# cheneeheng/2s-AGCN

Measured on AMD Instinct MI355X. Metric: skeleton-clips/sec fwd+bwd, NTU (N,3,300,25,2), higher is better.
Workload: dtype f32; 1 GPU; AGCN joint-stream NTU-xview shape, full training step (fwd, CE, bwd, grad all-reduce, clip 1.0, SGD nesterov); per_gpu_batch=64, global_batch=64, input=(N,3,300,25,2), parallelism=dp1, bn=per-replica

## Files before the change

2s-agcn_amd/csrc/wgrad9_bf16.hip:

```cpp
#include "agcn_common.h"
#include "split_bf16.h"
#include "split_f16.h"

namespace {

constexpr int TC = 80;
constexpr int DP = 84;
constexpr int XW = TC + 8;
constexpr int XPB = 88;

struct TrArgs {
  const float* in;
  float* out;
  int N, R, T, V, Tp, S;
  const float* absmax;
  long plane;
};

template <bool F16, int RB, int TT, int FPL>
__global__ void __launch_bounds__(256) tv_transpose_kernel(const TrArgs a) {
  extern __shared__ __attribute__((aligned(16))) float tile[];
  static_assert(FPL == 4 || (F16 && FPL == 8), "a lane writes one 16-byte store per plane");
  constexpr int QL = TT / FPL, NSUB = 64 / QL;
  const int S = a.S;
  const int ntt = (a.Tp * S + TT - 1) / TT, nrb = (a.R + RB - 1) / RB;
  int b = blockIdx.x;
  const int tti = b % ntt;
  b /= ntt;
  const int rb = b % nrb, n = b / nrb;
  const int t0 = tti * TT, r0 = rb * RB;
  const int tl = max(0, min(TT, a.T - t0));
  const int len = tl * a.V;
  const int pitch = TT * a.V + 4;
  const int lane = threadIdx.x & 63;
  const int wave = __builtin_amdgcn_readfirstlane(threadIdx.x >> 6);
  typedef const __attribute__((address_space(1))) void* gptr_t;
  typedef __attribute__((address_space(3))) void* lptr_t;
  const bool wide = ((a.T * a.V) & 3) == 0 && (len & 3) == 0 && len > 0 && ((reinterpret_cast<unsigned long>(a.in) & 15) == 0);
  if (wide) {
    const int npiece = (len + 255) >> 8;
    for (int p = wave; p < RB * npiece; p += 4) {
      const int r = p / npiece, e0 = (p - r * npiece) * 256;
      if (r0 + r < a.R) {
        const float* src = a.in + (((long)n * a.R + r0 + r) * a.T + t0) * a.V + e0;
        if (e0 + 4 * lane < len)
          __builtin_amdgcn_global_load_lds((gptr_t)(src + 4 * lane), (lptr_t)(tile + r * pitch + e0), 16, 0, 0);
      }
    }
  } else {
    const int npiece = (len + 63) >> 6;
    for (int p = wave; p < RB * npiece; p += 4) {
      const int r = p / npiece, e0 = (p - r * npiece) * 64;
      if (r0 + r < a.R) {
        const float* src = a.in + (((long)n * a.R + r0 + r) * a.T + t0) * a.V + e0;
        const int e = min(lane, len - 1 - e0);
        __builtin_amdgcn_global_load_lds((gptr_t)(src + e), (lptr_t)(tile + r * pitch + e0), 4, 0, 0);
      }
    }
  }
  __syncthreads();
  float rs_s = 1.f, rs_inv = 1.f;
  if constexpr (F16) f16_range_scale(a.absmax, rs_s, rs_inv);
  (void)rs_inv;
  const int TTo = TT / S;
  const int tw = min(TTo, a.Tp - t0 / S);
  const int qp = TTo / FPL;
  const int lq = lane % QL;
  const int par = lq / qp, q = lq - par * qp, sub = lane / QL;
  for (int p = wave * NSUB + sub; p < a.V * RB; p += 4 * NSUB) {
    const int v = p / RB, r = p - v * RB;
    if (r0 + r < a.R && FPL * q < tw) {
      float val[FPL];
#pragma unroll
      for (int j = 0; j < FPL; ++j) {
        const int f = (FPL * q + j) * S + par;
        val[j] = (f < tl) ? tile[r * pitch + f * a.V + v] : 0.f;
      }
      const long o = ((((long)n * a.V + v) * a.R + r0 + r) * S + par) * a.Tp + t0 / S + FPL * q;
      if constexpr (F16) {
        unsigned hh[FPL / 2], ll[FPL / 2];
#pragma unroll
        for (int j = 0; j < FPL / 2; ++j) split_pair_f16_mix(val[2 * j] * rs_s, val[2 * j + 1] * rs_s, hh[j], ll[j]);
        unsigned short* oh = reinterpret_cast<unsigned short*>(a.out);
        if constexpr (FPL == 8) {
          *reinterpret_cast<u32x4*>(oh + o) = u32x4{hh[0], hh[1], hh[2], hh[3]};
          *reinterpret_cast<u32x4*>(oh + a.plane + o) = u32x4{ll[0], ll[1], ll[2], ll[3]};
        } else {
          *reinterpret_cast<uint2*>(oh + o) = make_uint2(hh[0], hh[1]);
          *reinterpret_cast<uint2*>(oh + a.plane + o) = make_uint2(ll[0], ll[1]);
        }
      } else {
        *reinterpret_cast<f32x4*>(a.out + o) = f32x4{val[0], val[1], val[2], val[3]};
      }
    }
  }
}

struct W9Args {
  const float* dyT;
  const float* xT;
  float* part;
  int N, M, C, V, T, Tp;
  int nchunk, units, units_per_split, ncb;
  int npl;
  const unsigned short* dyH;
  const unsigned short* xH;
  long dy_plane, x_plane;
  const float* dy_absmax;
  const float* x_absmax;
};

template <int S>
__device__ __forceinline__ bf16x8 window_frag(const unsigned (&p)[8]) {
  u32x4 r;
  if (S % 2 == 0) {
#pragma unroll
    for (int i = 0; i < 4; ++i) r[i] = p[S / 2 + i];
  } else {
#pragma unroll
    for (int i = 0; i < 4; ++i) r[i] = __builtin_amdgcn_alignbit(p[(S + 1) / 2 + i], p[(S - 1) / 2 + i], 16);
  }
  return __builtin_bit_cast(bf16x8, r);
}

template <int S>
__device__ __forceinline__ f32x16 tap_mfma(bf16x8 a0, bf16x8 a1, bf16x8 a2, const unsigned (&p0)[8],
                                           const unsigned (&p1)[8], const unsigned (&p2)[8], f32x16 c, int npl) {
  return sb_mfma6(a0, a1, a2, window_frag<S>(p0), window_frag<S>(p1), window_frag<S>(p2), c, npl);
}

template <int RT, int CT, int STRIDE>
__global__ void __launch_bounds__(256, 2) wgrad9_bf16_kernel(const W9Args a) {
  constexpr int NT = 256, BM = RT * 32, CBW = CT * 32, SETS = STRIDE;
  static_assert(RT * CT == 4, "four waves");
  constexpr int ND = BM * (TC / 4) / NT;
  constexpr int NXG = CBW * SETS * (XW / 8);
  constexpr int NX = (NXG + NT - 1) / NT;
  static_assert(BM * (TC / 4) % NT == 0, "dy tile divides evenly");
  extern __shared__ __attribute__((aligned(16))) float smem[];
  float* dyL = smem;
  unsigned short* xP = reinterpret_cast<unsigned short*>(smem + BM * DP);
  const int tid = threadIdx.x, lane = tid & 63;
  const int wave = __builtin_amdgcn_readfirstlane(tid >> 6);
  const int lr = lane & 31, h = lane >> 5;
  const int rt = wave % RT, ct = wave / RT;
  const int mb = blockIdx.x / a.ncb, cb = blockIdx.x - mb * a.ncb;
  const int m0 = mb * BM, c0 = cb * CBW;
  const int split = blockIdx.y;
  const int u_begin = split * a.units_per_split;
  const int u_end = min(a.units, u_begin + a.units_per_split);
  const int Tp = a.Tp;

  f32x16 acc[9];
#pragma unroll
  for (int z = 0; z < 9; ++z)
#pragma unroll
    for (int j = 0; j < 16; ++j) acc[z][j] = 0.f;

  const float* arow = dyL + (rt * 32 + lr) * DP + 8 * h;
  const unsigned short* brow = xP + (ct * 32 + lr) * XPB + 8 * h;

  for (int unit = u_begin; unit < u_end; ++unit) {
    const int ch = unit % a.nchunk;
    const int nv = unit / a.nchunk;
    const int t0 = ch * TC;
    const float* src = a.dyT + ((long)nv * a.M + m0) * Tp + t0;
    const float* sx = a.xT + ((long)nv * a.C + c0) * SETS * Tp + (t0 - 4);
    int tv = tid;
    asm volatile("" : "+v"(tv));
    f32x4 dv[ND], xv[NX][2];
#pragma unroll
    for (int u = 0; u < ND; ++u) {
      const int i = tv + u * NT, r = i / (TC / 4), q = i - r * (TC / 4);
      const bool ok = (m0 + r < a.M) && (t0 + 4 * q < Tp);
      dv[u] = *reinterpret_cast<const f32x4*>(src + (ok ? r * Tp + 4 * q : 0));
      if (!ok) dv[u] = f32x4{0.f, 0.f, 0.f, 0.f};
    }
#pragma unroll
    for (int u = 0; u < NX; ++u) {
      const int i = min(tv + u * NT, NXG - 1), r = i / (XW / 8), k = i - r * (XW / 8);
#pragma unroll
      for (int hq = 0; hq < 2; ++hq) {
        const int t = t0 - 4 + 8 * k + 4 * hq;
        const bool ok = (c0 + r / SETS < a.C) && t >= 0 && t < Tp;
        xv[u][hq] = *reinterpret_cast<const f32x4*>(sx + (ok ? r * Tp + 8 * k + 4 * hq : 4));
        if (!ok) xv[u][hq] = f32x4{0.f, 0.f, 0.f, 0.f};
      }
    }
    __syncthreads();
    asm volatile("" : "+v"(tv));
#pragma unroll
    for (int u = 0; u < ND; ++u) {
      const int i = tv + u * NT, r = i / (TC / 4), q = i - r * (TC / 4);
      *reinterpret_cast<f32x4*>(dyL + r * DP + 4 * q) = dv[u];
    }
#pragma unroll
    for (int u = 0; u < NX; ++u) {
      const int i = min(tv + u * NT, NXG - 1), r = i / (XW / 8), k = i - r * (XW / 8);
      u32x4 ph, pm, pl;
#pragma unroll
      for (int e = 0; e < 4; ++e) {
        unsigned y0, y1, y2;
        sb_split_pair(xv[u][e >> 1][2 * (e & 1)], xv[u][e >> 1][2 * (e & 1) + 1], y0, y1, y2);
        ph[e] = y0; pm[e] = y1; pl[e] = y2;
      }
      const int row = (r % SETS) * CBW + r / SETS;
      *reinterpret_cast<u32x4*>(xP + (0 * SETS * CBW + row) * XPB + 8 * k) = ph;
      *reinterpret_cast<u32x4*>(xP + (1 * SETS * CBW + row) * XPB + 8 * k) = pm;
      *reinterpret_cast<u32x4*>(xP + (2 * SETS * CBW + row) * XPB + 8 * k) = pl;
    }
    __syncthreads();
#pragma unroll 1
    for (int ks = 0; ks < TC / 16; ++ks) {
      const f32x4 ar0 = *reinterpret_cast<const f32x4*>(arow + 16 * ks);
      const f32x4 ar1 = *reinterpret_cast<const f32x4*>(arow + 16 * ks + 4);
      u32x4 bw[SETS][3][2];
#pragma unroll
      for (int st = 0; st < SETS; ++st)
#pragma unroll
        for (int pl = 0; pl < 3; ++pl)
#pragma unroll
          for (int i = 0; i < 2; ++i)
            bw[st][pl][i] = *reinterpret_cast<const u32x4*>(brow + (pl * SETS + st) * CBW * XPB + 16 * ks + 8 * i);
      u32x4 ah, am, al;
      {
        unsigned x0, x1, x2;
        sb_split_pair(ar0[0], ar0[1], x0, x1, x2); ah[0] = x0; am[0] = x1; al[0] = x2;
        sb_split_pair(ar0[2], ar0[3], x0, x1, x2); ah[1] = x0; am[1] = x1; al[1] = x2;
        sb_split_pair(ar1[0], ar1[1], x0, x1, x2); ah[2] = x0; am[2] = x1; al[2] = x2;
        sb_split_pair(ar1[2], ar1[3], x0, x1, x2); ah[3] = x0; am[3] = x1; al[3] = x2;
      }
      unsigned p0[8], p1[8], p2[8], o0[8], o1[8], o2[8];
#pragma unroll
      for (int i = 0; i < 8; ++i) {
        p0[i] = bw[0][0][i >> 2][i & 3];
        p1[i] = bw[0][1][i >> 2][i & 3];
        p2[i] = bw[0][2][i >> 2][i & 3];
        o0[i] = bw[SETS - 1][0][i >> 2][i & 3];
        o1[i] = bw[SETS - 1][1][i >> 2][i & 3];
        o2[i] = bw[SETS - 1][2][i >> 2][i & 3];
      }
      const bf16x8 a0 = __builtin_bit_cast(bf16x8, ah), a1 = __builtin_bit_cast(bf16x8, am),
                   a2 = __builtin_bit_cast(bf16x8, al);
      if (STRIDE == 1) {
        acc[0] = tap_mfma<0>(a0, a1, a2, p0, p1, p2, acc[0], a.npl);
        acc[1] = tap_mfma<1>(a0, a1, a2, p0, p1, p2, acc[1], a.npl);
        acc[2] = tap_mfma<2>(a0, a1, a2, p0, p1, p2, acc[2], a.npl);
        acc[3] = tap_mfma<3>(a0, a1, a2, p0, p1, p2, acc[3], a.npl);
        acc[4] = tap_mfma<4>(a0, a1, a2, p0, p1, p2, acc[4], a.npl);
        acc[5] = tap_mfma<5>(a0, a1, a2, p0, p1, p2, acc[5], a.npl);
        acc[6] = tap_mfma<6>(a0, a1, a2, p0, p1, p2, acc[6], a.npl);
        acc[7] = tap_mfma<7>(a0, a1, a2, p0, p1, p2, acc[7], a.npl);
        acc[8] = tap_mfma<8>(a0, a1, a2, p0, p1, p2, acc[8], a.npl);
      } else {
        acc[0] = tap_mfma<2>(a0, a1, a2, p0, p1, p2, acc[0], a.npl);
        acc[1] = tap_mfma<2>(a0, a1, a2, o0, o1, o2, acc[1], a.npl);
        acc[2] = tap_mfma<3>(a0, a1, a2, p0, p1, p2, acc[2], a.npl);
        acc[3] = tap_mfma<3>(a0, a1, a2, o0, o1, o2, acc[3], a.npl);
        acc[4] = tap_mfma<4>(a0, a1, a2, p0, p1, p2, acc[4], a.npl);
        acc[5] = tap_mfma<4>(a0, a1, a2, o0, o1, o2, acc[5], a.npl);
        acc[6] = tap_mfma<5>(a0, a1, a2, p0, p1, p2, acc[6], a.npl);
        acc[7] = tap_mfma<5>(a0, a1, a2, o0, o1, o2, acc[7], a.npl);
        acc[8] = tap_mfma<6>(a0, a1, a2, p0, p1, p2, acc[8], a.npl);
      }
    }
  }

  float* dst = a.part + (long)split * 9 * a.M * a.C;
#pragma unroll
  for (int z = 0; z < 9; ++z)
#pragma unroll
    for (int j = 0; j < 16; ++j) {
      const int m = m0 + rt * 32 + mfma_row(j, h);
      const int c = c0 + ct * 32 + lr;
      if (m < a.M && c < a.C) dst[((long)z * a.M + m) * a.C + c] = acc[z][j];
    }
}


constexpr int DPH = 88;

template <int S>
__device__ __forceinline__ f32x16 tap_mfma_f16(f16x8 ah, f16x8 al, const unsigned (&ph)[8], const unsigned (&pl)[8],
                                               f32x16 c) {
  const f16x8 bh = __builtin_bit_cast(f16x8, window_frag<S>(ph)), bl = __builtin_bit_cast(f16x8, window_frag<S>(pl));
  c = __builtin_amdgcn_mfma_f32_32x32x16_f16(al, bh, c, 0, 0, 0);
  c = __builtin_amdgcn_mfma_f32_32x32x16_f16(ah, bl, c, 0, 0, 0);
  c = __builtin_amdgcn_mfma_f32_32x32x16_f16(ah, bh, c, 0, 0, 0);
  return c;
}

template <int RT, int CT, int STRIDE, int TAPS = 9, int SH0 = 0>
__global__ void __launch_bounds__(256, 2) wgrad9_f16_kernel(const W9Args a) {
  static_assert(STRIDE == 1 || (TAPS == 9 && SH0 == 0), "other tap counts at stride 1 only");
  static_assert(SH0 >= 0 && SH0 + TAPS - 1 <= 8, "every tap's 8 frames lie inside the 16-frame window");
  constexpr int NT = 256, BM = RT * 32, CBW = CT * 32, SETS = STRIDE;
  static_assert(RT * CT == 4, "four waves");
  constexpr int ND = BM * (TC / 4) / NT;
  constexpr int NXG = CBW * SETS * (XW / 8);
  constexpr int NX = (NXG + NT - 1) / NT;
  static_assert(BM * (TC / 4) % NT == 0, "dy tile divides evenly");
  extern __shared__ __attribute__((aligned(16))) unsigned short smh[];
  unsigned short* dyL = smh;
  unsigned short* xP = smh + 2 * BM * DPH;
  const int tid = threadIdx.x, lane = tid & 63;
  const int wave = __builtin_amdgcn_readfirstlane(tid >> 6);
  const int lr = lane & 31, h = lane >> 5;
  const int rt = wave % RT, ct = wave / RT;
  const int mb = blockIdx.x / a.ncb, cb = blockIdx.x - mb * a.ncb;
  const int m0 = mb * BM, c0 = cb * CBW;
  const int split = blockIdx.y;
  const int u_begin = split * a.units_per_split;
  const int u_end = min(a.units, u_begin + a.units_per_split);
  const int Tp = a.Tp;

  f32x16 acc[9];
#pragma unroll
  for (int z = 0; z < 9; ++z)
#pragma unroll
    for (int j = 0; j < 16; ++j) acc[z][j] = 0.f;

  const unsigned short* arow = dyL + (rt * 32 + lr) * DPH + 8 * h;
  const unsigned short* brow = xP + (ct * 32 + lr) * XPB + 8 * h;

  constexpr bool PREF = STRIDE == 1;
  uint2 dv[ND][2], xv[NX][2][2];
  auto fetch = [&](int unit) __attribute__((always_inline)) {
    const int ch = unit % a.nchunk;
    const int nv = unit / a.nchunk;
    const int t0 = ch * TC;
    const unsigned short* src = a.dyH + ((long)nv * a.M + m0) * Tp + t0;
    const unsigned short* sx = a.xH + ((long)nv * a.C + c0) * SETS * Tp + (t0 - 4);
    int tv = tid;
    asm volatile("" : "+v"(tv));
#pragma unroll
    for (int u = 0; u < ND; ++u) {
      const int i = tv + u * NT, r = i / (TC / 4), q = i - r * (TC / 4);
      const bool ok = (m0 + r < a.M) && (t0 + 4 * q < Tp);
      const int off = ok ? r * Tp + 4 * q : 0;
#pragma unroll
      for (int pl = 0; pl < 2; ++pl) {
        dv[u][pl] = *reinterpret_cast<const uint2*>(src + pl * a.dy_plane + off);
        if (!ok) dv[u][pl] = make_uint2(0u, 0u);
      }
    }
#pragma unroll
    for (int u = 0; u < NX; ++u) {
      const int i = min(tv + u * NT, NXG - 1), r = i / (XW / 8), k = i - r * (XW / 8);
#pragma unroll
      for (int hq = 0; hq < 2; ++hq) {
        const int t = t0 - 4 + 8 * k + 4 * hq;
        const bool ok = (c0 + r / SETS < a.C) && t >= 0 && t < Tp;
        const int off = ok ? r * Tp + 8 * k + 4 * hq : 4;
#pragma unroll
        for (int pl = 0; pl < 2; ++pl) {
          xv[u][hq][pl] = *reinterpret_cast<const uint2*>(sx + pl * a.x_plane + off);
          if (!ok) xv[u][hq][pl] = make_uint2(0u, 0u);
        }
      }
    }
  };
  if (PREF && u_begin < u_end) fetch(u_begin);
  for (int unit = u_begin; unit < u_end; ++unit) {
    if (!PREF) fetch(unit);
    __syncthreads();
    int tv = tid;
    asm volatile("" : "+v"(tv));
#pragma unroll
    for (int u = 0; u < ND; ++u) {
      const int i = tv + u * NT, r = i / (TC / 4), q = i - r * (TC / 4);
#pragma unroll
      for (int pl = 0; pl < 2; ++pl) *reinterpret_cast<uint2*>(dyL + (pl * BM + r) * DPH + 4 * q) = dv[u][pl];
    }
#pragma unroll
    for (int u = 0; u < NX; ++u) {
      const int i = min(tv + u * NT, NXG - 1), r = i / (XW / 8), k = i - r * (XW / 8);
      const int row = (r % SETS) * CBW + r / SETS;
#pragma unroll
      for (int hq = 0; hq < 2; ++hq)
#pragma unroll
        for (int pl = 0; pl < 2; ++pl)
          *reinterpret_cast<uint2*>(xP + (pl * SETS * CBW + row) * XPB + 8 * k + 4 * hq) = xv[u][hq][pl];
    }
    __syncthreads();
    if (PREF && unit + 1 < u_end) fetch(unit + 1);
#pragma unroll 1
    for (int ks = 0; ks < TC / 16; ++ks) {
      const f16x8 ah = *reinterpret_cast<const f16x8*>(arow + 16 * ks);
      const f16x8 al = *reinterpret_cast<const f16x8*>(arow + BM * DPH + 16 * ks);
      u32x4 bw[SETS][2][2];
#pragma unroll
      for (int st = 0; st < SETS; ++st)
#pragma unroll
        for (int pl = 0; pl < 2; ++pl)
#pragma unroll
          for (int i = 0; i < 2; ++i)
            bw[st][pl][i] = *reinterpret_cast<const u32x4*>(brow + (pl * SETS + st) * CBW * XPB + 16 * ks + 8 * i);
      unsigned p0[8], p1[8], o0[8], o1[8];
#pragma unroll
      for (int i = 0; i < 8; ++i) {
        p0[i] = bw[0][0][i >> 2][i & 3];
        p1[i] = bw[0][1][i >> 2][i & 3];
        o0[i] = bw[SETS - 1][0][i >> 2][i & 3];
        o1[i] = bw[SETS - 1][1][i >> 2][i & 3];
      }
      if constexpr (STRIDE == 1) {
        acc[0] = tap_mfma_f16<SH0 + 0>(ah, al, p0, p1, acc[0]);
        if constexpr (TAPS > 1) acc[1] = tap_mfma_f16<SH0 + 1>(ah, al, p0, p1, acc[1]);
        if constexpr (TAPS > 2) acc[2] = tap_mfma_f16<SH0 + 2>(ah, al, p0, p1, acc[2]);
        if constexpr (TAPS > 3) acc[3] = tap_mfma_f16<SH0 + 3>(ah, al, p0, p1, acc[3]);
        if constexpr (TAPS > 4) acc[4] = tap_mfma_f16<SH0 + 4>(ah, al, p0, p1, acc[4]);
        if constexpr (TAPS > 5) acc[5] = tap_mfma_f16<SH0 + 5>(ah, al, p0, p1, acc[5]);
        if constexpr (TAPS > 6) acc[6] = tap_mfma_f16<SH0 + 6>(ah, al, p0, p1, acc[6]);
        if constexpr (TAPS > 7) acc[7] = tap_mfma_f16<SH0 + 7>(ah, al, p0, p1, acc[7]);
        if constexpr (TAPS > 8) acc[8] = tap_mfma_f16<SH0 + 8>(ah, al, p0, p1, acc[8]);
      } else {
        acc[0] = tap_mfma_f16<2>(ah, al, p0, p1, acc[0]);
        acc[1] = tap_mfma_f16<2>(ah, al, o0, o1, acc[1]);
        acc[2] = tap_mfma_f16<3>(ah, al, p0, p1, acc[2]);
        acc[3] = tap_mfma_f16<3>(ah, al, o0, o1, acc[3]);
        acc[4] = tap_mfma_f16<4>(ah, al, p0, p1, acc[4]);
        acc[5] = tap_mfma_f16<4>(ah, al, o0, o1, acc[5]);
        acc[6] = tap_mfma_f16<5>(ah, al, p0, p1, acc[6]);
        acc[7] = tap_mfma_f16<5>(ah, al, o0, o1, acc[7]);
        acc[8] = tap_mfma_f16<6>(ah, al, p0, p1, acc[8]);
      }
    }
  }

  float s_dy, inv_dy, s_x, inv_x;
  f16_range_scale(a.dy_absmax, s_dy, inv_dy);
  f16_range_scale(a.x_absmax, s_x, inv_x);
  const float inv = inv_dy * inv_x;
  float* dst = a.part + (long)split * TAPS * a.M * a.C;
#pragma unroll
  for (int z = 0; z < TAPS; ++z)
#pragma unroll
    for (int j = 0; j < 16; ++j) {
      const int m = m0 + rt * 32 + mfma_row(j, h);
      const int c = c0 + ct * 32 + lr;
      if (m < a.M && c < a.C) dst[((long)z * a.M + m) * a.C + c] = acc[z][j] * inv;
    }
}

struct W9Geom {
  int Tp, nchunk, units, nmb, ncb, nsplit, units_per_split, rt;
  size_t slab_bytes, dyT_bytes, xT_bytes, smem_bytes, smem_f16;
};

inline W9Geom w9_geometry(int N, int M, int C, int V, int T, int stride, int taps = 9, int Tx = 0) {
  W9Geom g;
  g.rt = (M % 128 == 0) ? 4 : 2;
  const int BM = g.rt * 32, CBW = (4 / g.rt) * 32;
  g.Tp = ((Tx > T ? Tx : T) + 7) & ~7;
  g.nchunk = (T + TC - 1) / TC;
  g.units = N * V * g.nchunk;
  g.nmb = (M + BM - 1) / BM;
  g.ncb = (C + CBW - 1) / CBW;
  const int tiles = g.nmb * g.ncb;
  int want = 512 / tiles;
  if (want < 1) want = 1;
  if (want > g.units) want = g.units;
  g.units_per_split = (g.units + want - 1) / want;
  g.nsplit = (g.units + g.units_per_split - 1) / g.units_per_split;
  g.slab_bytes = (size_t)g.nsplit * taps * M * C * 4;
  g.dyT_bytes = (size_t)N * V * M * g.Tp * 4;
  g.xT_bytes = (size_t)N * V * C * stride * g.Tp * 4;
  g.smem_bytes = (size_t)BM * DP * 4 + (size_t)3 * stride * CBW * XPB * 2;
  g.smem_f16 = (size_t)2 * BM * DPH * 2 + (size_t)2 * stride * CBW * XPB * 2;
  return g;
}

int w9_transpose(const float* in, float* out, int N, int R, int T, int V, int Tp, int S, hipStream_t s,
                 const float* absmax = nullptr) {
  TrArgs t;
  t.in = in; t.out = out; t.N = N; t.R = R; t.T = T; t.V = V; t.Tp = Tp; t.S = S;
  t.absmax = absmax; t.plane = (long)N * V * R * S * Tp;
  if (absmax) {
    const int rem = T % 128;
    if (T <= 128 || rem == 0 || rem > 64) {
      constexpr int RB = 4, TT = 128;
      const int ntt = (Tp * S + TT - 1) / TT, nrb = (R + RB - 1) / RB;
      const size_t smem = (size_t)RB * (TT * V + 4) * 4;
      hipLaunchKernelGGL((tv_transpose_kernel<true, RB, TT, 8>), dim3((unsigned)(N * nrb * ntt)), dim3(256), smem, s, t);
    } else {
      constexpr int RB = 8, TT = 64;
      const int ntt = (Tp * S + TT - 1) / TT, nrb = (R + RB - 1) / RB;
      const size_t smem = (size_t)RB * (TT * V + 4) * 4;
      hipLaunchKernelGGL((tv_transpose_kernel<true, RB, TT, 8>), dim3((unsigned)(N * nrb * ntt)), dim3(256), smem, s, t);
    }
  } else {
    const int ntt = (Tp * S + 63) / 64, nrb = (R + 7) / 8;
    const size_t smem = (size_t)8 * (64 * V + 4) * 4;
    hipLaunchKernelGGL((tv_transpose_kernel<false, 8, 64, 4>), dim3((unsigned)(N * nrb * ntt)), dim3(256), smem, s, t);
  }
  return agcn_check_launch();
}

template <int RT, int CT, int STRIDE, int TAPS = 9, int SH0 = 0>
int w9_launch_f16(const W9Args& a, const W9Geom& g, hipStream_t s) {
  if (TAPS == 9) AGCN_NOTE_KERNEL("wgrad9_f16_kernel<%d, %d, %d>", RT, CT, STRIDE);
  else AGCN_NOTE_KERNEL("wgrad9_f16_kernel<%d, %d, %d, %d, %d>", RT, CT, STRIDE, TAPS, SH0);
  return agcn_launch_big<wgrad9_f16_kernel<RT, CT, STRIDE, TAPS, SH0>>(dim3((unsigned)(g.nmb * g.ncb), (unsigned)g.nsplit),
                                                                       dim3(256), g.smem_f16, s, a);
}

template <int RT, int CT, int STRIDE>
int w9_launch(const W9Args& a, const W9Geom& g, hipStream_t s) {
  AGCN_NOTE_KERNEL("wgrad9_bf16_kernel<%d, %d, %d>", RT, CT, STRIDE);
  return agcn_launch_big<wgrad9_bf16_kernel<RT, CT, STRIDE>>(dim3((unsigned)(g.nmb * g.ncb), (unsigned)g.nsplit), dim3(256),
                                                             g.smem_bytes, s, a);
}

template <int TAPS, int SH0>
int w9_launch_taps(const W9Args& a, const W9Geom& g, hipStream_t s) {
  return g.rt == 4 ? w9_launch_f16<4, 1, 1, TAPS, SH0>(a, g, s) : w9_launch_f16<2, 2, 1, TAPS, SH0>(a, g, s);
}

inline bool w9_f16x3() { return agcn_knob(AGCN_WGRAD9_F16X3) != 0; }

int w9_run(const float* dy, const float* x, void* ws, size_t ws_bytes, int* nslabs, int N, int M, int C, int V, int T,
           int taps, int stride, int pad, bool f16, const float* dy_absmax, const float* x_absmax, hipStream_t s,
           AgcnDryRun* dry) {
  const int To = (T + 2 * pad - taps) / stride + 1;
  if (To < 1 || (taps != 9 && !f16)) return AGCN_ERR_UNSUPPORTED;
  const W9Geom g = w9_geometry(N, M, C, V, To, stride, taps, taps == 9 ? 0 : T);
  const size_t bytes = g.slab_bytes + g.dyT_bytes + g.xT_bytes + 512;
  if (dry) return agcn_dry_note(dry, 0, bytes);
  if (bytes > ws_bytes) return AGCN_ERR_WORKSPACE;
  unsigned char* base = (unsigned char*)ws;
  float* dyT = (float*)(base + ((g.slab_bytes + 255) & ~(size_t)255));
  float* xT = (float*)((unsigned char*)dyT + g.dyT_bytes);
  if ((size_t)((unsigned char*)xT - base) + g.xT_bytes + 8 > ws_bytes) return AGCN_ERR_WORKSPACE;
  if (f16) {
    unsigned* scr = reinterpret_cast<unsigned*>((unsigned char*)xT + g.xT_bytes);
    if (int rc = agcn_operand_max(dy_absmax, dy, (long)N * M * To * V, scr, s, &dy_absmax)) return rc;
    if (int rc = agcn_operand_max(x_absmax, x, (long)N * C * T * V, scr + 1, s, &x_absmax)) return rc;
  }
  int rc = w9_transpose(dy, dyT, N, M, To, V, g.Tp, 1, s, f16 ? dy_absmax : nullptr);
  if (rc) return rc;
  rc = w9_transpose(x, xT, N, C, T, V, g.Tp, stride, s, f16 ? x_absmax : nullptr);
  if (rc) return rc;
  W9Args a = {};
  a.dyT = dyT; a.xT = xT; a.part = (float*)ws;
  a.N = N; a.M = M; a.C = C; a.V = V; a.T = To; a.Tp = g.Tp;
  a.nchunk = g.nchunk; a.units = g.units; a.units_per_split = g.units_per_split; a.ncb = g.ncb;
  a.npl = agcn_npl();
  *nslabs = g.nsplit;
  if (!f16) {
    if (stride == 2) return w9_launch<4, 1, 2>(a, g, s);
    return g.rt == 4 ? w9_launch<4, 1, 1>(a, g, s) : w9_launch<2, 2, 1>(a, g, s);
  }
  a.dyH = reinterpret_cast<const unsigned short*>(dyT);
  a.xH = reinterpret_cast<const unsigned short*>(xT);
  a.dy_plane = (long)N * V * M * g.Tp;
  a.x_plane = (long)N * V * C * stride * g.Tp;
  a.dy_absmax = dy_absmax; a.x_absmax = x_absmax;
  if (taps == 9) {
    if (stride == 2) return w9_launch_f16<4, 1, 2>(a, g, s);
    return g.rt == 4 ? w9_launch_f16<4, 1, 1>(a, g, s) : w9_launch_f16<2, 2, 1>(a, g, s);
  }
  switch (taps * 16 + 4 - pad) {
    case 3 * 16 + 3: return w9_launch_taps<3, 3>(a, g, s);
    case 3 * 16 + 4: return w9_launch_taps<3, 4>(a, g, s);
    case 5 * 16 + 2: return w9_launch_taps<5, 2>(a, g, s);
    case 5 * 16 + 3: return w9_launch_taps<5, 3>(a, g, s);
    case 5 * 16 + 4: return w9_launch_taps<5, 4>(a, g, s);
    case 7 * 16 + 1: return w9_launch_taps<7, 1>(a, g, s);
    case 7 * 16 + 2: return w9_launch_taps<7, 2>(a, g, s);
    default: return AGCN_ERR_UNSUPPORTED;
  }
}

}

bool agcn_wgrad9_bf16_supported(int M, int C, int V, int stride) {
  if (M % 64 != 0 || C % 64 != 0 || V < 1 || V > 32 || !agcn_chained()) return false;
  return stride == 1 || (stride == 2 && M % 128 == 0);
}

int agcn_wgrad9_bf16(const float* dy, const float* x, void* ws, size_t ws_bytes, int* nslabs, int N, int M, int C, int V,
                     int T, int stride, hipStream_t s, const float* dy_absmax, const float* x_absmax, AgcnDryRun* dry) {
  return w9_run(dy, x, ws, ws_bytes, nslabs, N, M, C, V, T, 9, stride, 4, agcn_npl() == 3 && w9_f16x3(), dy_absmax,
                x_absmax, s, dry);
}

bool agcn_wgrad_tconv_f16_supported(int M, int C, int V, int taps, int stride, int pad) {
  if (stride != 1 || (taps != 3 && taps != 5 && taps != 7) || pad < 0 || pad > (taps - 1) / 2 || taps - pad > 5)
    return false;
  return agcn_gemm_precision() == 3 && w9_f16x3() && M % 64 == 0 && C % 64 == 0 && V >= 1 && V <= 32;
}

int agcn_wgrad_tconv_f16(const float* dy, const float* x, void* ws, size_t ws_bytes, int* nslabs, int N, int M, int C,
                         int V, int T, int taps, int pad, hipStream_t s, const float* dy_absmax, const float* x_absmax,
                         AgcnDryRun* dry) {
  if (!agcn_wgrad_tconv_f16_supported(M, C, V, taps, 1, pad)) return AGCN_ERR_UNSUPPORTED;
  return w9_run(dy, x, ws, ws_bytes, nslabs, N, M, C, V, T, taps, 1, pad, true, dy_absmax, x_absmax, s, dry);
}
```

Baseline: 1028 clips/s.

## Add double-buffered global_load_lds wgrad9 f16 kernel with paired-plane layout

Adds a new temporal-conv weight-gradient kernel that streams dy and x tiles from global memory straight into LDS via global_load_lds. It double-buffers and spreads the next unit's loads across the first three k-steps so transfers overlap the MFMA work. The transpose now interleaves the hi/lo f16 planes per (n,v) row so one unit's data is contiguous, and a 128x64 tile shape is routed when C allows. The change adds LDS pressure (one block per CU via launch bounds), more complex addressing, and new routing checks that can return unsupported.

After: 1036 clips/s (median of 4 runs). About the same (+0.8%).

```diff
diff --git a/2s-agcn_amd/csrc/wgrad9_bf16.hip b/2s-agcn_amd/csrc/wgrad9_bf16.hip
--- a/2s-agcn_amd/csrc/wgrad9_bf16.hip
+++ b/2s-agcn_amd/csrc/wgrad9_bf16.hip
@@ -1,6 +1,8 @@
 #include "agcn_common.h"
 #include "split_bf16.h"
 #include "split_f16.h"
+#include "wgrad9_plan.h"
+#include <type_traits>
 
 namespace {
 
@@ -15,6 +17,7 @@
   int N, R, T, V, Tp, S;
   const float* absmax;
   long plane;
+  long nv_rows;
 };
 
 template <bool F16, int RB, int TT, int FPL>
@@ -76,7 +79,7 @@
         const int f = (FPL * q + j) * S + par;
         val[j] = (f < tl) ? tile[r * pitch + f * a.V + v] : 0.f;
       }
-      const long o = ((((long)n * a.V + v) * a.R + r0 + r) * S + par) * a.Tp + t0 / S + FPL * q;
+      const long o = ((((long)n * a.V + v) * a.nv_rows + r0 + r) * S + par) * a.Tp + t0 / S + FPL * q;
       if constexpr (F16) {
         unsigned hh[FPL / 2], ll[FPL / 2];
 #pragma unroll
@@ -443,39 +446,210 @@
     }
 }
 
+template <int STRIDE>
+struct W9Frags {
+  f16x8 ah, al;
+  u32x4 bw[STRIDE][2][2];
+};
+
+template <int RT, int CT, int STRIDE, int TAPS = 9, int SH0 = 0>
+__global__ void __launch_bounds__(RT * CT * 64, 1) wgrad9_f16_dma_kernel(const W9Args a) {
+  static_assert(STRIDE == 1 || (TAPS == 9 && SH0 == 0), "other tap counts at stride 1 only");
+  static_assert(SH0 >= 0 && SH0 + TAPS - 1 <= 8, "every tap's 8 frames lie inside the 16-frame window");
+  constexpr W9Carve CV = w9_carve(RT, CT, STRIDE);
+  static_assert(CV.lds_bytes <= W9_LDS_LIMIT, "two buffers fit the LDS");
+  constexpr int SETS = STRIDE, PER = CV.per_wave, ISSUE_STEPS = 3;
+  constexpr int PPS = (PER + ISSUE_STEPS - 1) / ISSUE_STEPS;
+  extern __shared__ __attribute__((aligned(16))) unsigned short smh[];
+  typedef const __attribute__((address_space(1))) void* gptr_t;
+  typedef __attribute__((address_space(3))) void* lptr_t;
+  const int tid = threadIdx.x, lane = tid & 63;
+  const int wave = __builtin_amdgcn_readfirstlane(tid >> 6);
+  const int lr = lane & 31, h = lane >> 5;
+  const int rt = wave % RT, ct = wave / RT;
+  const int mb = blockIdx.x / a.ncb, cb = blockIdx.x - mb * a.ncb;
+  const int m0 = mb * CV.bm, c0 = cb * CV.cbw;
+  const int split = blockIdx.y;
+  const int u_begin = split * a.units_per_split;
+  const int u_end = min(a.units, u_begin + a.units_per_split);
+
+  f32x16 acc[9];
+#pragma unroll
+  for (int z = 0; z < 9; ++z)
+#pragma unroll
+    for (int j = 0; j < 16; ++j) acc[z][j] = 0.f;
+
+  unsigned soff[PER];
+#pragma unroll
+  for (int i = 0; i < PER; ++i) {
+    const int w = max(w9_wave_instr(CV, wave, i), 0);
+    soff[i] = (unsigned)(2 * w9_piece(CV, w, lane, a.M, a.C, a.Tp).src_off);
+  }
+  const char* dyb = reinterpret_cast<const char*>(a.dyH);
+  const char* xb = reinterpret_cast<const char*>(a.xH);
+  char* lds = reinterpret_cast<char*>(smh);
+
+  const char *ud, *ux;
+  auto locate = [&](int unit) __attribute__((always_inline)) {
+    const int ch = unit % a.nchunk;
+    const long nv = unit / a.nchunk;
+    ud = dyb + 2 * w9_dy_unit(nv, a.M, m0, a.Tp, ch);
+    ux = xb + 2 * w9_x_unit(nv, a.C, c0, SETS, a.Tp, ch);
+  };
+  auto issue = [&](int b, auto I0, auto I1) __attribute__((always_inline)) {
+#pragma unroll
+    for (int i = decltype(I0)::value; i < decltype(I1)::value; ++i) {
+      const int w = w9_wave_instr(CV, wave, i);
+      const char* base = i < CV.dy_per_wave ? ud : ux;
+      unsigned so = soff[i];
+      asm volatile("" : "+v"(so));
+      if (w9_slot_full(CV, i) || w >= 0)
+        __builtin_amdgcn_global_load_lds((gptr_t)(base + so), (lptr_t)(lds + b * CV.buf_bytes + 1024 * w), 16, 0, 0);
+    }
+  };
+  auto frags = [&](int b, int ks) __attribute__((always_inline)) {
+    W9Frags<STRIDE> f;
+    const char* buf = lds + b * CV.buf_bytes;
+    f.ah = *reinterpret_cast<const f16x8*>(buf + w9_frag_a(CV, rt, lr, h, ks, 0));
+    f.al = *reinterpret_cast<const f16x8*>(buf + w9_frag_a(CV, rt, lr, h, ks, 1));
+#pragma unroll
+    for (int st = 0; st < SETS; ++st)
+#pragma unroll
+      for (int pl = 0; pl < 2; ++pl)
+#pragma unroll
+        for (int i = 0; i < 2; ++i)
+          f.bw[st][pl][i] = *reinterpret_cast<const u32x4*>(buf + w9_frag_b(CV, ct, lr, h, ks, pl, st, i));
+    return f;
+  };
+
+  if (u_begin < u_end) {
+    locate(u_begin);
+    issue(0, std::integral_constant<int, 0>(), std::integral_constant<int, PER>());
+  }
+  int b = 0;
+  for (int unit = u_begin; unit < u_end; ++unit, b ^= 1) {
+    asm volatile("s_waitcnt vmcnt(%0)" ::"n"(W9_VMCNT_AT_RETIRE) : "memory");
+    __builtin_amdgcn_s_barrier();
+    asm volatile("" ::: "memory");
+    const bool more = unit + 1 < u_end;
+    const int ch = unit % a.nchunk;
+    const int xlo = w9_x_lo(ch), xhi = w9_x_hi(ch, a.Tp), dhi = w9_dy_hi(ch, a.Tp);
+    if (more) locate(unit + 1);
+    constexpr bool FPRE = CV.nw == 4;
+    W9Frags<STRIDE> f;
+    if (FPRE) f = frags(b, 0);
+#pragma unroll
+    for (int ks = 0; ks < W9_KSTEPS; ++ks) {
+      W9Frags<STRIDE> fn;
+      if (FPRE && ks + 1 < W9_KSTEPS) fn = frags(b, ks + 1);
+      if (!FPRE) f = frags(b, ks);
+      if (more) {
+        if (ks == 0) issue(b ^ 1, std::integral_constant<int, 0>(), std::integral_constant<int, (PPS < PER ? PPS : PER)>());
+        if (ks == 1) issue(b ^ 1, std::integral_constant<int, (PPS < PER ? PPS : PER)>(), std::integral_constant<int, (2 * PPS < PER ? 2 * PPS : PER)>());
+        if (ks == 2) issue(b ^ 1, std::integral_constant<int, (2 * PPS < PER ? 2 * PPS : PER)>(), std::integral_constant<int, PER>());
+      }
+      unsigned p0[8], p1[8], o0[8], o1[8];
+#pragma unroll
+      for (int i = 0; i < 8; ++i) {
+        p0[i] = f.bw[0][0][i >> 2][i & 3];
+        p1[i] = f.bw[0][1][i >> 2][i & 3];
+        o0[i] = f.bw[SETS - 1][0][i >> 2][i & 3];
+        o1[i] = f.bw[SETS - 1][1][i >> 2][i & 3];
+      }
+      f16x8 ah = f.ah, al = f.al;
+      const int wf = w9_frag_first(h, ks);
+      if ((ks == 0 && xlo > 0) || 16 * ks + 24 > xhi) {
+#pragma unroll
+        for (int i = 0; i < 8; ++i) {
+          const bool ok = wf + 2 * i >= xlo && wf + 2 * i < xhi;
+          p0[i] = ok ? p0[i] : 0u; p1[i] = ok ? p1[i] : 0u;
+          o0[i] = ok ? o0[i] : 0u; o1[i] = ok ? o1[i] : 0u;
+        }
+      }
+      if (16 * ks + 16 > dhi && wf >= dhi) {
+#pragma unroll
+        for (int i = 0; i < 8; ++i) { ah[i] = 0; al[i] = 0; }
+      }
+      if constexpr (STRIDE == 1) {
+        acc[0] = tap_mfma_f16<SH0 + 0>(ah, al, p0, p1, acc[0]);
+        if constexpr (TAPS > 1) acc[1] = tap_mfma_f16<SH0 + 1>(ah, al, p0, p1, acc[1]);
+        if constexpr (TAPS > 2) acc[2] = tap_mfma_f16<SH0 + 2>(ah, al, p0, p1, acc[2]);
+        if constexpr (TAPS > 3) acc[3] = tap_mfma_f16<SH0 + 3>(ah, al, p0, p1, acc[3]);
+        if constexpr (TAPS > 4) acc[4] = tap_mfma_f16<SH0 + 4>(ah, al, p0, p1, acc[4]);
+        if constexpr (TAPS > 5) acc[5] = tap_mfma_f16<SH0 + 5>(ah, al, p0, p1, acc[5]);
+        if constexpr (TAPS > 6) acc[6] = tap_mfma_f16<SH0 + 6>(ah, al, p0, p1, acc[6]);
+        if constexpr (TAPS > 7) acc[7] = tap_mfma_f16<SH0 + 7>(ah, al, p0, p1, acc[7]);
+        if constexpr (TAPS > 8) acc[8] = tap_mfma_f16<SH0 + 8>(ah, al, p0, p1, acc[8]);
+      } else {
+        acc[0] = tap_mfma_f16<2>(ah, al, p0, p1, acc[0]);
+        acc[1] = tap_mfma_f16<2>(ah, al, o0, o1, acc[1]);
+        acc[2] = tap_mfma_f16<3>(ah, al, p0, p1, acc[2]);
+        acc[3] = tap_mfma_f16<3>(ah, al, o0, o1, acc[3]);
+        acc[4] = tap_mfma_f16<4>(ah, al, p0, p1, acc[4]);
+        acc[5] = tap_mfma_f16<4>(ah, al, o0, o1, acc[5]);
+        acc[6] = tap_mfma_f16<5>(ah, al, p0, p1, acc[6]);
+        acc[7] = tap_mfma_f16<5>(ah, al, o0, o1, acc[7]);
+        acc[8] = tap_mfma_f16<6>(ah, al, p0, p1, acc[8]);
+      }
+      if (FPRE && ks + 1 < W9_KSTEPS) f = fn;
+    }
+  }
+
+  float s_dy, inv_dy, s_x, inv_x;
+  f16_range_scale(a.dy_absmax, s_dy, inv_dy);
+  f16_range_scale(a.x_absmax, s_x, inv_x);
+  const float inv = inv_dy * inv_x;
+  float* dst = a.part + (long)split * TAPS * a.M * a.C;
+#pragma unroll
+  for (int z = 0; z < TAPS; ++z)
+#pragma unroll
+    for (int j = 0; j < 16; ++j) {
+      const int m = m0 + rt * 32 + mfma_row(j, h);
+      const int c = c0 + ct * 32 + lr;
+      if (m < a.M && c < a.C) dst[((long)z * a.M + m) * a.C + c] = acc[z][j] * inv;
+    }
+}
+
 struct W9Geom {
   int Tp, nchunk, units, nmb, ncb, nsplit, units_per_split, rt;
   size_t slab_bytes, dyT_bytes, xT_bytes, smem_bytes, smem_f16;
+  bool dma;
+  int ct;
 };
 
-inline W9Geom w9_geometry(int N, int M, int C, int V, int T, int stride, int taps = 9, int Tx = 0) {
+inline W9Geom w9_geometry(int N, int M, int C, int V, int T, int stride, int taps = 9, int Tx = 0, bool f16 = false) {
   W9Geom g;
   g.rt = (M % 128 == 0) ? 4 : 2;
+  const W9Route route = f16 ? w9_route(M, C, stride, taps) : W9Route{g.rt, 4 / g.rt, false};
+  g.dma = route.dma; g.ct = route.ct;
   const int BM = g.rt * 32, CBW = (4 / g.rt) * 32;
-  g.Tp = ((Tx > T ? Tx : T) + 7) & ~7;
+  g.Tp = w9_copy_pitch(T, Tx);
   g.nchunk = (T + TC - 1) / TC;
   g.units = N * V * g.nchunk;
   g.nmb = (M + BM - 1) / BM;
   g.ncb = (C + CBW - 1) / CBW;
   const int tiles = g.nmb * g.ncb;
-  int want = 512 / tiles;
-  if (want < 1) want = 1;
-  if (want > g.units) want = g.units;
-  g.units_per_split = (g.units + want - 1) / want;
-  g.nsplit = (g.units + g.units_per_split - 1) / g.units_per_split;
+  const W9Split sp = w9_split(g.units, tiles);
+  g.units_per_split = sp.units_per_split;
+  g.nsplit = sp.nsplit;
   g.slab_bytes = (size_t)g.nsplit * taps * M * C * 4;
   g.dyT_bytes = (size_t)N * V * M * g.Tp * 4;
   g.xT_bytes = (size_t)N * V * C * stride * g.Tp * 4;
   g.smem_bytes = (size_t)BM * DP * 4 + (size_t)3 * stride * CBW * XPB * 2;
   g.smem_f16 = (size_t)2 * BM * DPH * 2 + (size_t)2 * stride * CBW * XPB * 2;
+  if (g.dma) {
+    g.ncb = (C + g.ct * 32 - 1) / (g.ct * 32);
+    g.smem_f16 = (size_t)w9_carve(g.rt, g.ct, stride).lds_bytes;
+  }
   return g;
 }
 
 int w9_transpose(const float* in, float* out, int N, int R, int T, int V, int Tp, int S, hipStream_t s,
-                 const float* absmax = nullptr) {
+                 const float* absmax = nullptr, bool paired = false) {
   TrArgs t;
   t.in = in; t.out = out; t.N = N; t.R = R; t.T = T; t.V = V; t.Tp = Tp; t.S = S;
-  t.absmax = absmax; t.plane = (long)N * V * R * S * Tp;
+  t.absmax = absmax; t.plane = paired ? (long)R * S * Tp : (long)N * V * R * S * Tp;
+  t.nv_rows = paired ? 2L * R : R;
   if (absmax) {
     const int rem = T % 128;
     if (T <= 128 || rem == 0 || rem > 64) {
@@ -505,6 +679,14 @@
                                                                        dim3(256), g.smem_f16, s, a);
 }
 
+template <int RT, int CT, int STRIDE, int TAPS = 9, int SH0 = 0>
+int w9_launch_dma(const W9Args& a, const W9Geom& g, hipStream_t s) {
+  if (TAPS == 9) AGCN_NOTE_KERNEL("wgrad9_f16_kernel<%d, %d, %d>", RT, CT, STRIDE);
+  else AGCN_NOTE_KERNEL("wgrad9_f16_kernel<%d, %d, %d, %d, %d>", RT, CT, STRIDE, TAPS, SH0);
+  return agcn_launch_big<wgrad9_f16_dma_kernel<RT, CT, STRIDE, TAPS, SH0>>(
+      dim3((unsigned)(g.nmb * g.ncb), (unsigned)g.nsplit), dim3(RT * CT * 64), g.smem_f16, s, a);
+}
+
 template <int RT, int CT, int STRIDE>
 int w9_launch(const W9Args& a, const W9Geom& g, hipStream_t s) {
   AGCN_NOTE_KERNEL("wgrad9_bf16_kernel<%d, %d, %d>", RT, CT, STRIDE);
@@ -514,7 +696,7 @@
 
 template <int TAPS, int SH0>
 int w9_launch_taps(const W9Args& a, const W9Geom& g, hipStream_t s) {
-  return g.rt == 4 ? w9_launch_f16<4, 1, 1, TAPS, SH0>(a, g, s) : w9_launch_f16<2, 2, 1, TAPS, SH0>(a, g, s);
+  return g.rt == 4 ? w9_launch_dma<4, 1, 1, TAPS, SH0>(a, g, s) : w9_launch_f16<2, 2, 1, TAPS, SH0>(a, g, s);
 }
 
 inline bool w9_f16x3() { return agcn_knob(AGCN_WGRAD9_F16X3) != 0; }
@@ -524,8 +706,10 @@
            AgcnDryRun* dry) {
   const int To = (T + 2 * pad - taps) / stride + 1;
   if (To < 1 || (taps != 9 && !f16)) return AGCN_ERR_UNSUPPORTED;
-  const W9Geom g = w9_geometry(N, M, C, V, To, stride, taps, taps == 9 ? 0 : T);
-  const size_t bytes = g.slab_bytes + g.dyT_bytes + g.xT_bytes + 512;
+  const W9Geom g = w9_geometry(N, M, C, V, To, stride, taps, taps == 9 ? 0 : T, f16);
+  if (g.dma && (M % (g.rt * 32) != 0 || C % (g.ct * 32) != 0 || (stride == 2 && g.rt != 4) || V < 1))
+    return AGCN_ERR_UNSUPPORTED;
+  const size_t bytes = g.slab_bytes + g.dyT_bytes + g.xT_bytes + W9_WS_EXTRA;
   if (dry) return agcn_dry_note(dry, 0, bytes);
   if (bytes > ws_bytes) return AGCN_ERR_WORKSPACE;
   unsigned char* base = (unsigned char*)ws;
@@ -537,9 +721,9 @@
     if (int rc = agcn_operand_max(dy_absmax, dy, (long)N * M * To * V, scr, s, &dy_absmax)) return rc;
     if (int rc = agcn_operand_max(x_absmax, x, (long)N * C * T * V, scr + 1, s, &x_absmax)) return rc;
   }
-  int rc = w9_transpose(dy, dyT, N, M, To, V, g.Tp, 1, s, f16 ? dy_absmax : nullptr);
+  int rc = w9_transpose(dy, dyT, N, M, To, V, g.Tp, 1, s, f16 ? dy_absmax : nullptr, g.dma);
   if (rc) return rc;
-  rc = w9_transpose(x, xT, N, C, T, V, g.Tp, stride, s, f16 ? x_absmax : nullptr);
+  rc = w9_transpose(x, xT, N, C, T, V, g.Tp, stride, s, f16 ? x_absmax : nullptr, g.dma);
   if (rc) return rc;
   W9Args a = {};
   a.dyT = dyT; a.xT = xT; a.part = (float*)ws;
@@ -556,9 +740,11 @@
   a.dy_plane = (long)N * V * M * g.Tp;
   a.x_plane = (long)N * V * C * stride * g.Tp;
   a.dy_absmax = dy_absmax; a.x_absmax = x_absmax;
+  if (g.dma != (g.rt == 4 || taps == 9)) return AGCN_ERR_UNSUPPORTED;
   if (taps == 9) {
-    if (stride == 2) return w9_launch_f16<4, 1, 2>(a, g, s);
-    return g.rt == 4 ? w9_launch_f16<4, 1, 1>(a, g, s) : w9_launch_f16<2, 2, 1>(a, g, s);
+    if (stride == 2) return w9_launch_dma<4, 1, 2>(a, g, s);
+    if (g.rt == 4) return g.ct == 2 ? w9_launch_dma<4, 2, 1>(a, g, s) : w9_launch_dma<4, 1, 1>(a, g, s);
+    return w9_launch_dma<2, 2, 1>(a, g, s);
   }
   switch (taps * 16 + 4 - pad) {
     case 3 * 16 + 3: return w9_launch_taps<3, 3>(a, g, s);
diff --git a/2s-agcn_amd/csrc/wgrad9_plan.h b/2s-agcn_amd/csrc/wgrad9_plan.h
--- /dev/null
+++ b/2s-agcn_amd/csrc/wgrad9_plan.h
@@ -0,0 +1,128 @@
+#pragma once
+#include <cstddef>
+
+constexpr int W9_TC = 80;
+constexpr int W9_KSTEPS = W9_TC / 16;
+constexpr int W9_PITCH = 88;
+constexpr int W9_PPR = W9_PITCH / 8;
+constexpr int W9_BACK = 4;
+constexpr int W9_DY_PIECES = W9_TC / 8;
+constexpr int W9_LDS_LIMIT = 160 * 1024;
+constexpr int W9_TAIL_BYTES = 2 * (W9_PITCH - W9_BACK - 8);
+constexpr int W9_WS_EXTRA = 512;
+static_assert(W9_TAIL_BYTES + 256 <= W9_WS_EXTRA, "the tail of the last row's window stays inside the workspace");
+
+constexpr int w9_nchunk(int T) { return (T + W9_TC - 1) / W9_TC; }
+constexpr int w9_copy_pitch(int T, int Tx) { return ((Tx > T ? Tx : T) + 7) & ~7; }
+
+constexpr int w9_x_lo(int ch) { return ch == 0 ? W9_BACK : 0; }
+constexpr int w9_x_hi(int ch, int Tp) { return Tp - W9_TC * ch + W9_BACK < W9_PITCH ? Tp - W9_TC * ch + W9_BACK : W9_PITCH; }
+constexpr int w9_dy_hi(int ch, int Tp) { return Tp - W9_TC * ch < W9_TC ? Tp - W9_TC * ch : W9_TC; }
+constexpr bool w9_x_valid(int ch, int Tp, int w) { return w >= w9_x_lo(ch) && w < w9_x_hi(ch, Tp); }
+constexpr bool w9_dy_valid(int ch, int Tp, int f) { return f < w9_dy_hi(ch, Tp); }
+
+struct W9Carve {
+  int rt, ct, sets;
+  int nw, bm, cbw;
+  int dy_rows, x_rows;
+  int dy_instr, x_instr, instr;
+  int dy_per_wave, x_per_wave;
+  int per_wave;
+  int x_off, buf_bytes, lds_bytes;
+};
+
+constexpr W9Carve w9_carve(int rt, int ct, int stride) {
+  W9Carve c = {};
+  c.rt = rt; c.ct = ct; c.sets = stride;
+  c.nw = rt * ct; c.bm = rt * 32; c.cbw = ct * 32;
+  c.dy_rows = 2 * c.bm; c.x_rows = 2 * c.sets * c.cbw;
+  c.dy_instr = c.dy_rows * W9_PPR / 64; c.x_instr = c.x_rows * W9_PPR / 64;
+  c.instr = c.dy_instr + c.x_instr;
+  c.dy_per_wave = (c.dy_instr + c.nw - 1) / c.nw; c.x_per_wave = (c.x_instr + c.nw - 1) / c.nw;
+  c.per_wave = c.dy_per_wave + c.x_per_wave;
+  c.x_off = c.dy_rows * W9_PITCH * 2;
+  c.buf_bytes = (c.dy_rows + c.x_rows) * W9_PITCH * 2;
+  c.lds_bytes = 2 * c.buf_bytes;
+  return c;
+}
+
+constexpr W9Carve W9_C128x64 = w9_carve(4, 2, 1);
+constexpr W9Carve W9_C128x32 = w9_carve(4, 1, 1);
+constexpr W9Carve W9_C64x64 = w9_carve(2, 2, 1);
+constexpr W9Carve W9_C128x32S2 = w9_carve(4, 1, 2);
+static_assert(W9_C128x64.lds_bytes <= W9_LDS_LIMIT && W9_C128x32.lds_bytes <= W9_LDS_LIMIT &&
+              W9_C64x64.lds_bytes <= W9_LDS_LIMIT && W9_C128x32S2.lds_bytes <= W9_LDS_LIMIT, "two buffers fit the LDS");
+
+constexpr int w9_wave_instr(const W9Carve& c, int wave, int i) {
+  if (i < c.dy_per_wave) return i * c.nw + wave < c.dy_instr ? i * c.nw + wave : -1;
+  const int w = c.dy_instr + (i - c.dy_per_wave) * c.nw + wave;
+  return w < c.instr ? w : -1;
+}
+constexpr bool w9_slot_full(const W9Carve& c, int i) { return w9_wave_instr(c, c.nw - 1, i) >= 0; }
+constexpr int W9_VMCNT_AT_RETIRE = 0;
+
+struct W9Piece {
+  bool x;
+  int plane, row;
+  int first;
+  int lds_off;
+  long src_off;
+};
+
+constexpr W9Piece w9_piece(const W9Carve& c, int w, int lane, int M, int C, int Tp) {
+  W9Piece p = {};
+  const int q = 64 * w + lane;
+  p.lds_off = 16 * q;
+  if (w < c.dy_instr) {
+    const int r = q / W9_PPR, j = q - r * W9_PPR;
+    p.x = false; p.plane = r / c.bm; p.row = r - p.plane * c.bm;
+    p.first = j < W9_DY_PIECES ? 8 * j : -1;
+    p.src_off = ((long)p.plane * M + p.row) * Tp + 8 * (j < W9_DY_PIECES ? j : W9_DY_PIECES - 1);
+  } else {
+    const int qx = q - 64 * c.dy_instr;
+    const int r = qx / W9_PPR, j = qx - r * W9_PPR;
+    p.x = true; p.plane = r / (c.sets * c.cbw); p.row = r - p.plane * (c.sets * c.cbw);
+    p.first = 8 * j;
+    const int set = p.row / c.cbw, ch = p.row - set * c.cbw;
+    p.src_off = (((long)p.plane * C + ch) * c.sets + set) * Tp + 8 * j;
+  }
+  return p;
+}
+
+constexpr long w9_dy_unit(long nv, int M, int m0, int Tp, int ch) { return (nv * 2 * M + m0) * Tp + W9_TC * ch; }
+constexpr long w9_x_unit(long nv, int C, int c0, int sets, int Tp, int ch) {
+  return (nv * 2 * C + c0) * sets * Tp + W9_TC * ch - W9_BACK;
+}
+constexpr size_t w9_dy_copy_elems(long NV, int M, int Tp) { return (size_t)NV * 2 * M * Tp; }
+constexpr size_t w9_x_copy_elems(long NV, int C, int sets, int Tp) { return (size_t)NV * 2 * C * sets * Tp; }
+
+constexpr int w9_frag_first(int h, int ks) { return 16 * ks + 8 * h; }
+constexpr int w9_frag_a(const W9Carve& c, int rt, int lr, int h, int ks, int plane) {
+  return ((plane * c.bm + rt * 32 + lr) * W9_PITCH + w9_frag_first(h, ks)) * 2;
+}
+constexpr int w9_frag_b(const W9Carve& c, int ct, int lr, int h, int ks, int plane, int set, int i) {
+  return c.x_off + (((plane * c.sets + set) * c.cbw + ct * 32 + lr) * W9_PITCH + w9_frag_first(h, ks) + 8 * i) * 2;
+}
+
+struct W9Split {
+  int units_per_split, nsplit;
+};
+constexpr W9Split w9_split(int units, int tiles4) {
+  int want = 512 / tiles4;
+  if (want < 1) want = 1;
+  if (want > units) want = units;
+  W9Split s = {};
+  s.units_per_split = (units + want - 1) / want;
+  s.nsplit = (units + s.units_per_split - 1) / s.units_per_split;
+  return s;
+}
+
+struct W9Route {
+  int rt, ct;
+  bool dma;
+};
+constexpr W9Route w9_route(int M, int C, int stride, int taps) {
+  if (stride == 2) return {4, 1, true};
+  if (M % 128 == 0) return {4, taps == 9 && C % 64 == 0 ? 2 : 1, true};
+  return {2, 2, taps == 9};
+}
```
